# firechecking/CleanTransformer

Measured on AMD Instinct MI355X. Metric: SFT tokens/sec/step Bloom-560M bf16, higher is better.
Workload: dtype bf16

## Files before the change

cleantransformer_amd/_lib.py:

```python
from __future__ import annotations

import ctypes as C
import os

import torch

from ._build import LIB_PATH as _DEFAULT_LIB_PATH

LIB_PATH = os.environ.get("CTMI_LIB_PATH") or _DEFAULT_LIB_PATH

F32, BF16, F16 = 0, 1, 2
OPT_LEGACY_GRID = 4
OPT_SHADOW_F16 = 2
EPI_NONE, EPI_GELU, EPI_DGELU, EPI_RELU, EPI_DRELU, EPI_GELUG, EPI_MUL = 0, 1, 2, 3, 4, 5, 6
MT_MAX = 24
PROF_CLASSES = ("gemm_fwd", "gemm_dgrad", "gemm_wgrad", "lm_head", "attn_fwd", "attn_bwd", "layernorm", "loss", "optimizer", "reduce", "other")
ABI_VERSION = 16

vp, i64, i32, f32 = C.c_void_p, C.c_int64, C.c_int, C.c_float


class CtmiError(RuntimeError):
    pass


class AttnDesc(C.Structure):
    _fields_ = [(n, i64) for n in ("B", "nh", "Sq", "Sk", "hd",
                                   "q_bs", "q_hs", "q_rs", "k_bs", "k_hs", "k_rs",
                                   "v_bs", "v_hs", "v_rs", "o_bs", "o_hs", "o_rs",
                                   "am_b", "am_h", "am_q", "am_k")] + [("scale", f32), ("causal", i32), ("future_fill", f32), ("dropout_seed", C.c_uint32), ("dropout_p", f32), ("reserved_", i32)]


# ... 4 lines not shown
class WgradProblem(C.Structure):
    _fields_ = [("dy", vp), ("x", vp), ("dw", vp), ("db", vp), ("n_out", i64), ("n_in", i64), ("in_out", i32), ("pad_", i32)]


BLK_SLOTS = ("ln1", "mean1", "rstd1", "qkv", "att", "stat_m", "stat_l", "h1", "mean2", "rstd2", "ln2", "u", "g", "out")
BLK_QKV_BLOCKED, BLK_WGRAD_IN_OUT, BLK_W_IN_OUT = 1, 2, 4
BLK_PARAMS = ("ln1_w", "ln1_b", "wqkv", "bqkv", "wd", "bd", "ln2_w", "ln2_b", "w1", "b1", "w2", "b2")


class BloomBlock(C.Structure):
    _fields_ = [("B", i64), ("S", i64), ("H", i64), ("nh", i64), ("eps", f32), ("post_ln_res", i32), ("dtype", i32), ("flags", i32),
                ("attn_scale", f32), ("future_fill", f32)] + \
               [(n, vp) for n in BLK_PARAMS] + [(n, vp) for n in ("slopes", "kpos", "kvalid", "first_valid", "x", "slab")]


class BloomBlockGrads(C.Structure):
    _fields_ = [("dout", vp), ("dx", vp)] + [("d" + n, vp) for n in BLK_PARAMS] + \
               [("ws", vp), ("ws_bytes", i64), ("splitk_ws", vp), ("splitk_ws_bytes", i64), ("side_stream", vp),
                ("side_splitk_ws", vp), ("side_splitk_ws_bytes", i64), ("defer_join", i32)]


PROTOTYPES = {
    "ctmi_abi_version": (i32, []),
    "ctmi_last_error": (C.c_char_p, []),
    "ctmi_layernorm_fwd": (i32, [vp, vp, vp, vp, vp, vp, i64, i64, f32, i32, vp]),
    "ctmi_layernorm_bwd_ws": (i64, [i64, i64]),
    "ctmi_layernorm_bwd": (i32, [vp, vp, vp, vp, vp, vp, vp, vp, vp, i32, vp, i64, i64, i32, vp]),
    "ctmi_gemm": (i32, [vp, i64, i32, vp, i64, i32, vp, i64, i64, i64, i64, f32, i32, vp, vp, i32, vp, vp, i32, i32, vp, i64, vp]),
    "ctmi_set_launch_policy": (i32, [i32, i32]),
    "ctmi_get_launch_policy": (i32, [C.POINTER(i32), C.POINTER(i32)]),
    "ctmi_colsum": (i32, [vp, i64, vp, i32, vp, i64, i64, i32, vp]),
    "ctmi_colsum_ws": (i64, [i64, i64]),
    "ctmi_attn_fwd": (i32, [vp, vp, vp, vp, vp, vp, vp, vp, vp, vp, vp, C.POINTER(AttnDesc), i32, vp]),
    "ctmi_attn_bwd": (i32, [vp, vp, vp, vp, vp, vp, vp, vp, vp, vp, vp, vp, vp, vp, vp, vp, C.POINTER(AttnDesc), i32, vp]),
# ... 1 lines not shown
    "ctmi_mask_prep": (i32, [vp, vp, vp, vp, i64, i64, vp]),
    "ctmi_embed_fwd": (i32, [vp, vp, vp, i64, i64, i64, i32, vp, vp]),
    "ctmi_embed_bwd": (i32, [vp, vp, vp, i64, i64, i64, i32, f32, vp]),
    "ctmi_ce_fwd": (i32, [vp, i64, vp, vp, vp, vp, i64, i64, i64, i64, i64, i32, i64, i32, vp]),
    "ctmi_ce_bwd": (i32, [vp, i64, vp, vp, vp, vp, vp, i64, i64, i64, i64, i64, i64, i32, vp]),
    "ctmi_ce_fwd_bwd": (i32, [vp, i64, vp, vp, vp, vp, vp, i64, i64, i64, i64, i64, i64, i32, i64, f32, vp, i32, vp]),
    "ctmi_scale_if": (i32, [vp, i64, i64, i64, vp, f32, vp, i32, vp]),
    "ctmi_scale_if_passes": (i64, []),
    "ctmi_reduce_jobs": (i32, [C.POINTER(ReduceJob), i32, vp]),
    "ctmi_wgrad_grouped": (i32, [C.POINTER(WgradProblem), i32, i64, i32, vp, i64, vp]),
    "ctmi_bloom_block_layout": (i64, [i64, i64, i64, i64, i32, C.POINTER(i64)]),
    "ctmi_bloom_block_fwd": (i32, [C.POINTER(BloomBlock), vp]),
    "ctmi_bloom_block_bwd_ws": (i64, [i64, i64, i64, i64, i32]),
    "ctmi_bloom_block_wgrad_grouped": (i32, [i64, i64, i64, i32, i32]),
    "ctmi_bloom_block_bwd": (i32, [C.POINTER(BloomBlock), C.POINTER(BloomBlockGrads), vp]),
    "ctmi_ce_soft_fwd": (i32, [vp, i64, vp, i64, vp, vp, vp, vp, i64, i64, i32, i64, i32, vp]),
    "ctmi_ce_soft_bwd": (i32, [vp, i64, vp, i64, vp, vp, vp, vp, vp, i64, i64, i64, i32, vp]),
    "ctmi_ddp_unique_id": (C.c_int, [C.c_void_p]),
    "ctmi_ddp_create": (C.c_int, [C.c_void_p, C.c_int, C.c_int, C.c_int, C.POINTER(C.c_void_p)]),
    "ctmi_ddp_destroy": (C.c_int, [C.c_void_p]),
    "ctmi_ddp_all_reduce": (C.c_int, [C.c_void_p, C.c_void_p, C.c_int64, C.c_int, C.c_void_p]),
    "ctmi_ddp_all_gather": (C.c_int, [C.c_void_p, C.c_void_p, C.c_void_p, C.c_int64, C.c_void_p]),
    "ctmi_ddp_broadcast": (C.c_int, [C.c_void_p, C.c_void_p, C.c_int64, C.c_int, C.c_void_p]),
    "ctmi_ddp_wait": (C.c_int, [C.c_void_p, C.c_void_p]),
    "ctmi_dropout_hash": (C.c_uint32, [C.c_uint32]),
    "ctmi_dropout_keep_hash": (C.c_uint32, [C.c_uint32, C.c_uint32]),
    "ctmi_dropout_threshold": (C.c_uint32, [f32]),
    "ctmi_dropout": (i32, [vp, vp, vp, i64, f32, C.c_uint32, i32, vp]),
    "ctmi_adamw_step": (i32, [C.POINTER(vp), C.POINTER(vp), C.POINTER(vp), C.POINTER(vp), C.POINTER(vp), C.POINTER(i64),
                              i32, f32, f32, f32, f32, f32, i32, i32, i32, f32, vp]),
# ... 63 lines not shown
```

cleantransformer_amd/csrc/block.hip:

```cpp
#include "common.h"
#include <math.h>
#include <stdlib.h>
#include <mutex>

int ctmi_ln_bwd_parts_internal(const void* dy, const void* x, const float* w, const float* mean, const float* rstd,
                               const void* dres, void* dx, float* ws, int64_t rows, int64_t cols, int dtype, int want_sums,
                               int* nparts, int* ns, hipStream_t st);
int ctmi_colsum_parts_internal(const void* x, int64_t ld, float* ws, int64_t M, int64_t N, int dtype, int* parts_out, hipStream_t st);
bool ctmi_wgrad_grouped_ok(const ctmi_wgrad_problem* pr, int n, int64_t T, int dtype);
int ctmi_wgrad_grouped_ex(const ctmi_wgrad_problem* pr, int n, int64_t T, int dtype, void* workspace, int64_t workspace_bytes, void* stream, bool defer_reduce);
int ctmi_wgrad_tail(const ctmi_reduce_job* jobs, int count, hipStream_t st);
void ctmi_wgrad_pending_clear();
bool ctmi_wgrad_pending();

static inline int64_t al256(int64_t b) { return (b + 255) / 256 * 256; }

extern "C" int64_t ctmi_bloom_block_layout(int64_t B, int64_t S, int64_t H, int64_t nh, int dtype, int64_t* offs) {
    const int64_t T = B * S, e = dtype == CTMI_F32 ? 4 : 2;
    int64_t o = 0;
    auto put = [&](int slot, int64_t bytes) { if (offs) offs[slot] = o; o += al256(bytes); };
    put(CTMI_BLK_LN1, T * H * e);
    put(CTMI_BLK_MEAN1, T * 4);
    put(CTMI_BLK_RSTD1, T * 4);
    put(CTMI_BLK_QKV, T * 3 * H * e);
    put(CTMI_BLK_ATT, T * H * e);
// ... 135 lines not shown
}
}

extern "C" int ctmi_bloom_block_wgrad_grouped(int64_t B, int64_t S, int64_t H, int dtype, int flags) {
    if (B <= 0 || S <= 0 || H <= 0) return 0;
    const int io = (flags & CTMI_BLK_WGRAD_IN_OUT) ? 1 : 0;
    void* const al = reinterpret_cast<void*>(uintptr_t(256));
    float* const fa = reinterpret_cast<float*>(al);
    const ctmi_wgrad_problem wp[4] = {{al, al, fa, nullptr, H, 4 * H, io, 0}, {al, al, fa, io ? nullptr : fa, 4 * H, H, io, 0},
                                      {al, al, fa, nullptr, H, H, io, 0}, {al, al, fa, io ? nullptr : fa, 3 * H, H, io, 0}};
    return ctmi_wgrad_grouped_ok(wp, 4, B * S, dtype) ? 1 : 0;
}

extern "C" int64_t ctmi_bloom_block_bwd_ws(int64_t B, int64_t S, int64_t H, int64_t nh, int dtype) {
    return bwd_layout(B, S, H, nh, dtype, nullptr);
}

extern "C" int ctmi_bloom_block_bwd(const ctmi_bloom_block* b, const ctmi_bloom_block_grads* gr, void* stream) {
    RC(check_block(b, "bloom_block_bwd"));
    CTMI_REQUIRE(gr != nullptr && gr->dout && gr->dx && gr->ws, "bloom_block_bwd: null gradient pointer / workspace");
    CTMI_REQUIRE(gr->dln1_w && gr->dln1_b && gr->dwqkv && gr->dbqkv && gr->dwd && gr->dbd && gr->dln2_w && gr->dln2_b && gr->dw1 && gr->db1 &&
                 gr->dw2 && gr->db2, "bloom_block_bwd: null parameter-gradient pointer");
    const int64_t T = b->B * b->S, H = b->H, hd = H / b->nh;
    const int dt = b->dtype, e = dt == CTMI_F32 ? 4 : 2;
    int64_t woff[W_NSLOTS];
    const int64_t need = bwd_layout(b->B, b->S, H, b->nh, dt, woff);
    CTMI_REQUIRE(gr->ws_bytes >= need, "bloom_block_bwd: workspace too small (%lld < %lld bytes)", (long long)gr->ws_bytes, (long long)need);
    Slab s; s.base = reinterpret_cast<char*>(b->slab);
    ctmi_bloom_block_layout(b->B, b->S, H, b->nh, dt, s.off);
    char* wsb = reinterpret_cast<char*>(gr->ws);
// ... 6 lines not shown
    hipStream_t side = gr->side_stream ? as_stream(gr->side_stream) : nullptr;
    const bool two = side != nullptr && side != main_st;
    hipStream_t pst = two ? side : main_st;
    void* pws = two ? gr->side_splitk_ws : gr->splitk_ws;
    const int64_t pws_bytes = two ? gr->side_splitk_ws_bytes : gr->splitk_ws_bytes;
    auto fork = [&]() -> int {
        if (!two) return CTMI_OK;
        hipEvent_t ev = next_event();
        CTMI_HIP_OK(hipEventRecord(ev, main_st), "bloom_block_bwd: event record");
        CTMI_HIP_OK(hipStreamWaitEvent(side, ev, 0), "bloom_block_bwd: stream wait");
        return CTMI_OK;
    };

    ctmi_wgrad_pending_clear();
    ctmi_reduce_job jobs[CTMI_REDUCE_MAX_JOBS];
    int nj = 0;
    auto job = [&](const float* src, int64_t stride, int nparts, float* dst, int64_t n) {
        ctmi_reduce_job& J = jobs[nj++];
        J.src = src; J.dst = dst; J.n = n; J.part_stride = stride; J.nparts = nparts; J.accumulate = 0; J.alpha = 1.0f; J.pad_ = 0;
    };
    auto colsum_job = [&](const void* x, int64_t N, int slot, float* dst) -> int {
        int parts = 0;
        RC(ctmi_colsum_parts_internal(x, N, WF(slot), T, N, dt, &parts, pst));
        job(WF(slot), N, parts, dst, N);
        return CTMI_OK;
    };

    const void* dout = gr->dout;
    ctmi_wgrad_problem wp[4] = {
        {dout, s.at(CTMI_BLK_G), gr->dw2, nullptr, H, 4 * H, wio ? 1 : 0, 0},
        {W(W_DU), s.at(CTMI_BLK_LN2), gr->dw1, gr->db1, 4 * H, H, wio ? 1 : 0, 0},
        {W(W_DH1), s.at(CTMI_BLK_ATT), gr->dwd, nullptr, H, H, wio ? 1 : 0, 0},
        {W(W_DQKV), s.at(CTMI_BLK_LN1), gr->dwqkv, gr->dbqkv, 3 * H, H, wio ? 1 : 0, 0},
    };
    const int wp_cs[4] = {-1, W_CS_DU, -1, W_CS_DQKV};
    const bool grouped = ctmi_wgrad_grouped_ok(wp, 4, T, dt);
    int np2 = 0, ns2 = 2;
    auto out_bias_jobs = [&]() -> int {
        if (ns2 == 4 && !post) job(WF(W_LNP2) + 2 * H, ns2 * H, np2, gr->db2, H);
        else RC(colsum_job(dout, H, W_CS_DOUT, gr->db2));
        if (ns2 == 4) job(WF(W_LNP2) + 3 * H, ns2 * H, np2, gr->dbd, H);
        else RC(colsum_job(W(W_DH1), H, W_CS_DH1, gr->dbd));
        return CTMI_OK;
    };
    auto wgrad = [&](int i) -> int {
        if (grouped) return CTMI_OK;
        RC(fork());
        if (i == 2) RC(out_bias_jobs());
        const ctmi_wgrad_problem& p = wp[i];
        RC(linear_wgrad(p.dy, p.x, p.dw, T, p.n_out, p.n_in, dt, pws, pws_bytes, pst, wio));
        if (p.db) RC(colsum_job(p.dy, p.n_out, wp_cs[i], p.db));
// ... 7 lines not shown
        RC(ctmi_ln_bwd_parts_internal(W(W_DLN2), s.at(CTMI_BLK_H1), b->ln2_w, s.at<float>(CTMI_BLK_MEAN2), s.at<float>(CTMI_BLK_RSTD2),
                                      post ? nullptr : dout, W(W_DH1), WF(W_LNP2), T, H, dt, 1, &np2, &ns2, main_st));
        job(WF(W_LNP2), ns2 * H, np2, gr->dln2_w, H);
        job(WF(W_LNP2) + H, ns2 * H, np2, gr->dln2_b, H);
        RC(wgrad(2));
        RC(linear_dgrad(W(W_DH1), b->wd, W(W_DATT), T, H, H, CTMI_EPI_NONE, nullptr, nullptr, dt, gr->splitk_ws, gr->splitk_ws_bytes, main_st, w_io));
        const ctmi_attn_desc d = fused_qkv_desc(b);
        char* qkv = s.at<char>(CTMI_BLK_QKV);
        char* dqkv = reinterpret_cast<char*>(W(W_DQKV));
        RC(ctmi_attn_bwd(qkv, qkv + qkv_part(b, 1) * e, qkv + qkv_part(b, 2) * e, s.at(CTMI_BLK_ATT), W(W_DATT), s.at<float>(CTMI_BLK_STAT_M), s.at<float>(CTMI_BLK_STAT_L),
                         dqkv, dqkv + qkv_part(b, 1) * e, dqkv + qkv_part(b, 2) * e, WF(W_DELTA), b->slopes, b->kpos, b->kvalid, b->first_valid, nullptr, &d, dt, main_st));
        RC(wgrad(3));
        if (grouped) {
            RC(fork());
            RC(out_bias_jobs());
            RC(ctmi_wgrad_grouped_ex(wp, 4, T, dt, pws, pws_bytes, pst, !two));
        }
        const bool pend = ctmi_wgrad_pending();
        RC(linear_dgrad(dqkv, b->wqkv, W(W_DLN1), T, 3 * H, H, CTMI_EPI_NONE, nullptr, post ? W(W_DH1) : nullptr, dt, pend ? nullptr : gr->splitk_ws, pend ? 0 : gr->splitk_ws_bytes, main_st, w_io));
        int np1 = 0, ns1 = 2;
        RC(ctmi_ln_bwd_parts_internal(W(W_DLN1), b->x, b->ln1_w, s.at<float>(CTMI_BLK_MEAN1), s.at<float>(CTMI_BLK_RSTD1),
                                      post ? nullptr : W(W_DH1), gr->dx, WF(W_LNP1), T, H, dt, 0, &np1, &ns1, main_st));
        job(WF(W_LNP1), ns1 * H, np1, gr->dln1_w, H);
        job(WF(W_LNP1) + H, ns1 * H, np1, gr->dln1_b, H);
        return CTMI_OK;
    }();
    if (two && gr->defer_join && rc_launch == CTMI_OK) {
        RC(fork());
        RC(ctmi_reduce_jobs(jobs, nj, side));
        return CTMI_OK;
    }
    if (two) {
        hipEvent_t ev = next_event();
        const hipError_t e1 = hipEventRecord(ev, side);
        const hipError_t e2 = e1 == hipSuccess ? hipStreamWaitEvent(main_st, ev, 0) : e1;
        if (e2 != hipSuccess && rc_launch == CTMI_OK) { ctmi_set_error("bloom_block_bwd: joining the side stream: %s", hipGetErrorString(e2)); return CTMI_ERR_LAUNCH; }
    }
    if (rc_launch != CTMI_OK) { ctmi_wgrad_pending_clear(); return rc_launch; }
    RC(ctmi_wgrad_tail(jobs, nj, main_st));
    return CTMI_OK;
}
```

cleantransformer_amd/csrc/gemm.hip:

```cpp
#include "common.h"
#include "reduce_jobs.h"
#include <type_traits>
#include "mma.h"
#include "prof.h"
#include <atomic>
#ifndef CTMI_GEMM_PART
#define CTMI_GEMM_PART (-1)
#endif
#define CTMI_GEMM_HAS(p) (CTMI_GEMM_PART == -1 || CTMI_GEMM_PART == (p))

constexpr bool glds_k2(bool pp, int wm) { return pp && wm == 4; }
constexpr int glds_ring(bool pp, int wm, bool xlane = false) { return !pp ? 3 : (glds_k2(pp, wm) ? 6 : 4); }
constexpr int glds_patch_bytes(bool pp, int wm, bool xlane = false) { return (pp && !xlane && wm != 4) ? 4 * 8192 : 0; }


template <typename T> struct Tile;
template <> struct Tile<bf16_t> { static constexpr int BM = 128, BN = 128, BK = 64, PADK = 8, PADR = 8; };
template <> struct Tile<f16_t>  { static constexpr int BM = 128, BN = 128, BK = 64, PADK = 8, PADR = 8; };
template <> struct Tile<float>  { static constexpr int BM = 128, BN = 128, BK = 16, PADK = 4, PADR = 4; };

template <typename T, bool KMAJOR, int ROWS>
struct OpTile {
    static constexpr int BK = Tile<T>::BK;
    static constexpr int VEC = 16 / sizeof(T);
// ... 92 lines not shown
template <> __device__ __forceinline__ float OpTile<float, true, 128>::frag(const float* __restrict__ tile, int r16, int lane, int kofs) {
    return tile[kofs * PITCH + r16 + (lane & 15)];
}

struct GemmArgs {
    const void* A; const void* B; void* C;
    int64_t lda, ldb, ldc, M, N, K;
    float alpha; int beta;
    const float* bias; const void* residual; const void* aux_in; void* aux_out;
    int tiles_m, tiles_n, vec_c, vec8;
    int nt_c;
    int splits; int64_t k_per_split; float* slabs;
    int splitk_ok; float* ws; int64_t ws_bytes;
};

constexpr int WG_MAXP = 4;
struct GroupProb { const void* A; const void* B; float* C; float* cs; float* part; float* cspart; int64_t lda, ldb, ldc, M, N, csn; };
struct GroupedArgs : GemmArgs { GroupProb p[WG_MAXP]; const int4* items; int nitems; };
constexpr int WG_PART = 16, WG_COLSUM = 32, WG_HALF1 = 64, WG_COLSUMB = 128;
template <bool GRP, int WM, bool BSUM = false> struct GrpRegs { };
template <int WM> struct GrpRegs<true, WM, false> { f32x4 accs; bool cs_on; };
template <int WM> struct GrpRegs<true, WM, true> { f32x4 accs; bool cs_on; f32x4 accb[4]; bool csb_on; };
#define WG_ONES8 (std::is_same<T, f16_t>::value ? short8{0x3C00, 0x3C00, 0x3C00, 0x3C00, 0x3C00, 0x3C00, 0x3C00, 0x3C00} \
                                                : short8{0x3F80, 0x3F80, 0x3F80, 0x3F80, 0x3F80, 0x3F80, 0x3F80, 0x3F80})

template <typename TO> __device__ __forceinline__ void store4(TO* p, const float* v);
template <> __device__ __forceinline__ void store4<float>(float* p, const float* v) { *reinterpret_cast<float4*>(p) = make_float4(v[0], v[1], v[2], v[3]); }
template <> __device__ __forceinline__ void store4<bf16_t>(bf16_t* p, const float* v) { *reinterpret_cast<uint2*>(p) = make_uint2(pack_bf2(v[0], v[1]), pack_bf2(v[2], v[3])); }
template <> __device__ __forceinline__ void store4<f16_t>(f16_t* p, const float* v) { *reinterpret_cast<uint2*>(p) = make_uint2(pack_h2(v[0], v[1]), pack_h2(v[2], v[3])); }
template <typename TO> __device__ __forceinline__ void load4(const TO* p, float* v);
template <> __device__ __forceinline__ void load4<float>(const float* p, float* v) { float4 t = *reinterpret_cast<const float4*>(p); v[0] = t.x; v[1] = t.y; v[2] = t.z; v[3] = t.w; }
template <> __device__ __forceinline__ void load4<bf16_t>(const bf16_t* p, float* v) {
    uint2 t = *reinterpret_cast<const uint2*>(p);
    v[0] = __uint_as_float(t.x << 16); v[1] = __uint_as_float(t.x & 0xffff0000u); v[2] = __uint_as_float(t.y << 16); v[3] = __uint_as_float(t.y & 0xffff0000u);
// ... 1197 lines not shown
}

#if CTMI_GEMM_HAS(1)
int ctmi_gemm_bf16_nt(GemmArgs& g, int epi, bool fast, hipStream_t st) { return gemm_nt<bf16_t, bf16_t>(g, epi, fast, st); }
#endif
#if CTMI_GEMM_HAS(2)
int ctmi_gemm_bf16_nn(GemmArgs& g, int epi, bool fast, hipStream_t st) { return gemm_nn<bf16_t, bf16_t>(g, epi, fast, st); }
#endif
#if CTMI_GEMM_HAS(3)
int ctmi_gemm_bf16_tn(GemmArgs& g, int epi, bool fast, hipStream_t st) { return gemm_tn<bf16_t>(g, epi, fast, st); }

#include <map>
#include <mutex>
#include <vector>
namespace {
struct WgShape { int64_t M[WG_MAXP], N[WG_MAXP]; int cs[WG_MAXP]; int n; int64_t ksteps; int slots; int split;
    bool operator<(const WgShape& o) const {
        if (n != o.n) return n < o.n;
        if (ksteps != o.ksteps) return ksteps < o.ksteps;
        if (slots != o.slots) return slots < o.slots;
        if (split != o.split) return split < o.split;
        for (int i = 0; i < n; ++i) { if (M[i] != o.M[i]) return M[i] < o.M[i]; if (N[i] != o.N[i]) return N[i] < o.N[i]; if (cs[i] != o.cs[i]) return cs[i] < o.cs[i]; }
        return false;
    }
};
struct WgTable { int4* dev = nullptr; int nitems = 0, nsplit = 0; unsigned split_mask = 0; };
std::mutex g_wg_mu;
std::map<std::pair<int, WgShape>, WgTable> g_wg_tables;

inline int xcd_pos(int b, int L) {
    const int xcd = b & 7, q = L >> 3, r8 = L & 7;
    return (xcd < r8 ? xcd * (q + 1) : r8 * (q + 1) + (xcd - r8) * q) + (b >> 3);
}

void build_items(const WgShape& sh, std::vector<int4>& out, int& nitems, int& nsplit, unsigned& split_mask) {
    struct Tile { int p, m0, n0; };
    std::vector<Tile> tiles;
    for (int p = 0; p < sh.n; ++p) {
        const int tm = (int)(sh.M[p] / 128), tn = (int)(sh.N[p] / 256);
        for (int g0 = 0; g0 < tm; g0 += 8) {
            const int gm = std::min(8, tm - g0);
            for (int j = 0; j < tn; ++j)
                for (int i = 0; i < gm; ++i) tiles.push_back({p, (g0 + i) * 128, j * 256});
        }
    }
    const int nt = (int)tiles.size(), slots = sh.slots;
    const int ks = (int)sh.ksteps, h0 = ks / 2, h1 = ks - h0;
    int whole = nt;
    if (sh.split == 2 && ks >= 2) whole = 0;
    else if (sh.split == 1 && ks >= 2) { const int R = nt % slots; if (R > 0 && 2 * R <= slots) whole = nt - R; }
    split_mask = 0;
    auto csflag = [&](const Tile& t) { return sh.cs[t.p] == 1 ? (t.n0 == 0 ? WG_COLSUM : 0) : (sh.cs[t.p] == 2 ? (t.m0 == 0 ? WG_COLSUMB : 0) : 0); };
    auto item = [&](const Tile& t, int kb, int n, bool part) {
        const int cs = csflag(t);
        if (part) split_mask |= 1u << t.p;
        return make_int4(t.p | (part ? WG_PART : 0) | ((part && kb) ? WG_HALF1 : 0) | cs, t.m0, t.n0, kb | (n << 16));
    };
    std::vector<int4> lin;
    for (int t = 0; t < whole; ++t) lin.push_back(item(tiles[t], 0, ks, false));
    for (int t0 = whole; t0 < nt; t0 += 16) {
        const int t1 = std::min(nt, t0 + 16);
        for (int t = t0; t < t1; ++t) lin.push_back(item(tiles[t], 0, h0, true));
        for (int t = t0; t < t1; ++t) lin.push_back(item(tiles[t], h0, h1, true));
    }
    const int total = (int)lin.size();
    out.assign(total, make_int4(0, 0, 0, 0));
    for (int r0 = 0; r0 < total; r0 += slots) {
        const int L = std::min(slots, total - r0);
        for (int b = 0; b < L; ++b) out[r0 + b] = lin[r0 + xcd_pos(b, L)];
    }
    nitems = total; nsplit = nt - whole;
    for (int t = whole; t < nt; ++t) out.push_back(make_int4(tiles[t].p | csflag(tiles[t]), tiles[t].m0, tiles[t].n0, 0));
}
}

int ctmi_wgrad_group_mode() {
    static const int v = std::max(0, ctmi_env_int("CTMI_WGRAD_GROUP", 1));
    return v;
}

bool ctmi_wgrad_grouped_ok(const ctmi_wgrad_problem* pr, int n, int64_t T, int dtype) {
    if (ctmi_wgrad_group_mode() == 0 || !glds_enabled() || (dtype != CTMI_BF16 && dtype != CTMI_F16) || n < 1 || n > WG_MAXP || T < 64 || T % 32 != 0 || T / 32 > 0x7fff) return false;
    for (int i = 0; i < n; ++i) {
        const int64_t M = pr[i].in_out ? pr[i].n_in : pr[i].n_out, N = pr[i].in_out ? pr[i].n_out : pr[i].n_in;
        if (M <= 0 || N <= 0 || M % 128 != 0 || N % 256 != 0) return false;
        if (M * N >= (32LL << 20)) return false;
        if (!pr[i].dy || !pr[i].x || !pr[i].dw) return false;
        if ((((uintptr_t)pr[i].dy) | ((uintptr_t)pr[i].x) | ((uintptr_t)pr[i].dw)) & 15) return false;
// ... 9 lines not shown
    if (!g_wg_pending.valid) return ctmi_reduce_jobs(jobs, count, st);
    g_wg_pending.valid = false;
    if (st != g_wg_pending.st || count > CTMI_REDUCE_MAX_JOBS || count <= 0) {
        hipLaunchKernelGGL(wgrad_partials_reduce_k, dim3(4 * g_wg_pending.z.ntiles), dim3(256), 0, g_wg_pending.st, g_wg_pending.z);
        CTMI_CHECK_LAUNCH("wgrad_grouped_reduce");
        return ctmi_reduce_jobs(jobs, count, st);
    }
    ProfScope prof__(CTMI_PROF_REDUCE, st);
    ReduceJobs R;
    const int chunks = reduce_jobs_pack(jobs, count, R);
    if (chunks < 0) return CTMI_ERR_ARG;
    hipLaunchKernelGGL(wgrad_tail_k, dim3((unsigned)(4 * g_wg_pending.z.ntiles + chunks)), dim3(256), 0, st, g_wg_pending.z, R);
    CTMI_CHECK_LAUNCH("wgrad_tail");
    return CTMI_OK;
}
int ctmi_wgrad_grouped_ex(const ctmi_wgrad_problem* pr, int n, int64_t T, int dtype, void* workspace, int64_t workspace_bytes, void* stream, bool defer_reduce);
extern "C" int ctmi_wgrad_grouped(const ctmi_wgrad_problem* pr, int n, int64_t T, int dtype, void* workspace, int64_t workspace_bytes, void* stream) {
    return ctmi_wgrad_grouped_ex(pr, n, T, dtype, workspace, workspace_bytes, stream, false);
}
int ctmi_wgrad_grouped_ex(const ctmi_wgrad_problem* pr, int n, int64_t T, int dtype, void* workspace, int64_t workspace_bytes, void* stream, bool defer_reduce) {
    CTMI_REQUIRE(pr != nullptr, "wgrad_grouped: null problem list");
    if (!ctmi_wgrad_grouped_ok(pr, n, T, dtype)) {
        ctmi_set_error("wgrad_grouped: unsupported problem set (bf16 / fp16, <= %d problems, rows a multiple of 128 and columns of 256 of every gradient, T %% 32 == 0, "
                       "16-byte aligned operands and bias gradients; CTMI_WGRAD_GROUP != 0)", WG_MAXP);
        return CTMI_ERR_UNSUPPORTED;
    }
    hipStream_t st = as_stream(stream);
    ProfScope prof__(CTMI_PROF_GEMM_WGRAD, st);
    const int persist = shared_mode() ? 0 : 1;
    const int slots = (256 - reserved_cus()) / 8 * 8;
    WgShape sh = {};
    sh.n = n; sh.ksteps = T / 32; sh.slots = slots;
    const int mode = ctmi_wgrad_group_mode();
    sh.split = mode == 3 ? 0 : (mode == 2 ? 2 : 1);
    {
        int64_t need = 0;
        for (int i = 0; i < n; ++i) { const int64_t M = pr[i].in_out ? pr[i].n_in : pr[i].n_out, N = pr[i].in_out ? pr[i].n_out : pr[i].n_in; need += 2 * (M * N + std::max(M, N)) * 4 + 512; }
        if (sh.split != 0 && (workspace == nullptr || workspace_bytes < need || (((uintptr_t)workspace) & 15))) {
            static std::atomic<bool> said{false};
            if (!said.exchange(true))
                fprintf(stderr, "[ctmi355] wgrad_grouped: workspace of %lld bytes (need %lld, 16-byte aligned) — the tiles of the last partial round are NOT cut "
                                "in K-halves (same results, lower speed)\n", (long long)workspace_bytes, (long long)need);
            sh.split = 0;
        }
    }
    GroupedArgs g = {};
    bool bsum = false;
    g.M = 128; g.N = 256; g.K = T; g.k_per_split = T; g.splits = 1; g.alpha = 1.0f;
    for (int i = 0; i < n; ++i) {
// ... 138 lines not shown
```

cleantransformer_amd/models/modeling_bloom.py:

```python
from __future__ import annotations

import math
import os as _os
from typing import NamedTuple, Optional

import torch

from .. import _lib, ops, rng
from ..generation.generation_util import GenerationMixin
from ..transformer import LayerNorm

Tensor = torch.Tensor


class BloomConfig():

    def __init__(
            self,
            vocab_size=250880,
            hidden_size=64,
            n_layer=2,
            num_attention_heads=8,
            layer_norm_epsilon=1e-5,
            initializer_range=0.02,
# ... 84 lines not shown
                                   flags=spec.flags, attn_scale=spec.attn_scale, future_fill=spec.future_fill)
        ops.note_block_params(spec.mask, ps)
        grad = getattr(kv_out, "grad", True) and any(ctx.needs_input_grad)
        if grad:
            ctx.save_for_backward(x2, *ps, acts.slab)
            ctx.geo, ctx.spec, ctx.shape = acts.geometry(), spec, (B, S, H)
        kv = ops.LazyKV(acts, blocked=spec.kv_blocked, eager=not grad)
        if grad:
            ctx.kv = kv
        kv_out.append(kv)
        return acts.out.view(B, S, H)

    @staticmethod
    def backward(ctx, dout):
        if dout is None:
            return (None,) * (1 + _NP + 2)
        x2, *ps, slab = ctx.saved_tensors
        spec = ctx.spec
        B, S, H = ctx.shape
        dout2 = ops._c(dout.reshape(B * S, H))
        ctx.kv.release()
        side = _WGRAD_SIDE_STREAM if spec.side_stream_override else None
        defer = side is not False and x2.is_cuda and ops.params_allow_deferred_grads(ps, spec.mask)
        dx, g = ops.bloom_block_bwd(ops.BlockActs.rebuild(slab, ctx.geo), x2, ops.block_params(ps, x2.dtype), spec.mask, spec.slopes, spec.eps,
                                    spec.post_ln_res, dout2, use_side_stream=side, defer_join=defer)
        return (dx.view(B, S, H), *g, None, None)


def _lora_of(linear: torch.nn.Module):
    a = getattr(linear, "lora_A", None)
    return None if a is None else (a.weight, linear.lora_B.weight, float(linear.lora_scaling))


def _project(x2: Tensor, w_c: Tensor, bias: Tensor, res: Optional[Tensor], lora, p: float = 0.0, seed: int = 0):
    y = ops.linear_fwd(x2, w_c, bias, residual=None if p > 0.0 else res)
    xa = None
    if lora is not None:
        a, b, scaling = lora
        a_c, b_c = ops.compute_weight(a, x2.dtype), ops.compute_weight(b, x2.dtype)
        xa = ops.lora_project(x2, a_c, False, alpha=scaling)
# ... 444 lines not shown
```

cleantransformer_amd/ops.py:

```python
from __future__ import annotations

import contextlib
import os
import ctypes as C
import math
import threading
from typing import Optional, Tuple

import torch

from . import _lib
from ._lib import AttnDesc, BF16, F16, F32, check

Tensor = torch.Tensor


def _p(t: Optional[Tensor]):
    return None if t is None else C.c_void_p(t.data_ptr())


def _stream():
    return C.c_void_p(torch.cuda.current_stream().cuda_stream)


# ... 568 lines not shown


_GROUPED = {}
_WGRAD_STREAM_ENV = os.environ.get("CTMI_WGRAD_STREAM", "auto")


def block_wgrad_grouped(B: int, S: int, H: int, dtype: torch.dtype, flags: int = 0) -> bool:
    key = (B, S, H, dtype, flags)
    v = _GROUPED.get(key)
    if v is None:
        v = bool(_lib.load().ctmi_bloom_block_wgrad_grouped(B, S, H, dt_code(dtype), int(flags)))
        _GROUPED[key] = v
    return v


def bloom_block_bwd(acts: BlockActs, x2: Tensor, params, mask: Optional[MaskInfo], slopes: Optional[Tensor], eps: float,
                    post_ln_res: bool, dout2: Tensor, use_side_stream: Optional[bool] = None, defer_join: bool = False):
    _need_cuda(x2, dout2)
    B, S, H, nh = acts.B, acts.S, acts.H, acts.nh
    dev = x2.device
    if use_side_stream is None:
        use_side_stream = (_WGRAD_STREAM_ENV != "0") if _WGRAD_STREAM_ENV in ("0", "1") else not block_wgrad_grouped(B, S, H, x2.dtype, acts.flags)
    if torch.cuda.is_current_stream_capturing():
        use_side_stream = defer_join = False
    d = _lib.BloomBlock()
    _fill_block_desc(d, x2, params, mask, slopes, eps, post_ln_res, B, S, H, nh, acts.slab, acts.flags, acts.attn_scale, acts.future_fill)
    g = _lib.BloomBlockGrads()
    dx = torch.empty_like(x2)
    flip = bool(acts.flags & _lib.BLK_WGRAD_IN_OUT) != bool(acts.flags & _lib.BLK_W_IN_OUT)
    grads = [torch.empty(tuple(reversed(p.shape)) if (flip and p.dim() == 2) else p.shape, dtype=torch.float32, device=dev) for p in params]
    g.dout, g.dx = dout2.data_ptr(), dx.data_ptr()
    for name, t in zip(_lib.BLK_PARAMS, grads):
        setattr(g, "d" + name, t.data_ptr())
    defer_join = bool(defer_join and use_side_stream)
    main = torch.cuda.current_stream(dev)
    st = None
    slot = 0
    if defer_join:
        st = _DEFER.setdefault(dev, [0, {}])
        slot = st[0]
        st[0] ^= 1
        prev = st[1].get(slot)
        if prev is not None:
            main.wait_event(prev)
    elif dev in _DEFER and _DEFER[dev][1] and not torch.cuda.is_current_stream_capturing():
        for ev in _DEFER[dev][1].values():
            main.wait_event(ev)
        _DEFER[dev][1].clear()
    ws = _block_ws(dev, acts.lay.bwd_ws_bytes, slot)
    g.ws, g.ws_bytes = ws.data_ptr(), ws.numel()
    sk = _splitk_ws(dev)
    g.splitk_ws, g.splitk_ws_bytes = sk.data_ptr(), sk.numel() * 4
    if use_side_stream:
        side = side_stream(dev)
        with torch.cuda.stream(side):
            sk2 = _splitk_ws(dev)
        g.side_stream = side.cuda_stream
        g.side_splitk_ws, g.side_splitk_ws_bytes = sk2.data_ptr(), sk2.numel() * 4
    g.defer_join = int(defer_join)
    check(_lib.load().ctmi_bloom_block_bwd(C.byref(d), C.byref(g), _stream()), "bloom_block_bwd")
    if defer_join:
        ev = torch.cuda.Event()
        ev.record(side)
        st[1][slot] = ev
        acts.slab.record_stream(side)
        dout2.record_stream(side)
        for t in grads:
            t.record_stream(side)
        _LAST_DEFERRED_GRAD_PTRS[:] = [t.data_ptr() for t in grads]
        torch.autograd.Variable._execution_engine.queue_callback(lambda main=main, side=side: main.wait_stream(side))
    return dx, grads


def dropout(x: Tensor, p: float, seed: int, residual: Optional[Tensor] = None, out: Optional[Tensor] = None) -> Tensor:
    _need_cuda(x, residual)
# ... 385 lines not shown
```

include/ctmi355.h:

```cpp
#ifndef CTMI355_H
#define CTMI355_H

#include <stdint.h>

#ifdef __cplusplus
extern "C" {
#endif

#define CTMI_ABI_VERSION 16

enum ctmi_dtype { CTMI_F32 = 0, CTMI_BF16 = 1, CTMI_F16 = 2 };
enum ctmi_status { CTMI_OK = 0, CTMI_ERR_ARG = -1, CTMI_ERR_LAUNCH = -2, CTMI_ERR_UNSUPPORTED = -3 };

int ctmi_abi_version(void);
const char* ctmi_last_error(void);

int ctmi_layernorm_fwd(const void* x, const float* w, const float* b, void* y, float* mean, float* rstd,
                       int64_t rows, int64_t cols, float eps, int dtype, void* stream);
int64_t ctmi_layernorm_bwd_ws(int64_t rows, int64_t cols);
int ctmi_layernorm_bwd(const void* dy, const void* x, const float* w, const float* mean, const float* rstd,
                       const void* dres, void* dx, float* dw, float* db, int accumulate, float* ws,
                       int64_t rows, int64_t cols, int dtype, void* stream);

enum ctmi_epilogue { CTMI_EPI_NONE = 0, CTMI_EPI_GELU = 1, CTMI_EPI_DGELU = 2, CTMI_EPI_RELU = 3, CTMI_EPI_DRELU = 4,
// ... 144 lines not shown
    float eps; int32_t post_ln_res;
    int32_t dtype;
    int32_t flags;
    float attn_scale;
    float future_fill;
    const float *ln1_w, *ln1_b; const void* wqkv; const float* bqkv; const void* wd; const float* bd;
    const float *ln2_w, *ln2_b; const void* w1; const float* b1; const void* w2; const float* b2;
    const float* slopes;
    const float* kpos; const int32_t* kvalid; const int32_t* first_valid;
    const void* x;
    void* slab;
} ctmi_bloom_block;
int64_t ctmi_bloom_block_layout(int64_t B, int64_t S, int64_t H, int64_t nh, int dtype, int64_t* offsets );
int ctmi_bloom_block_fwd(const ctmi_bloom_block* blk , void* stream);

typedef struct ctmi_bloom_block_grads {
    const void* dout;
    void* dx;
    float *dln1_w, *dln1_b, *dwqkv, *dbqkv, *dwd, *dbd, *dln2_w, *dln2_b, *dw1, *db1, *dw2, *db2;
    void* ws; int64_t ws_bytes;
    void* splitk_ws; int64_t splitk_ws_bytes;
    void* side_stream;
    void* side_splitk_ws; int64_t side_splitk_ws_bytes;
    int defer_join;
} ctmi_bloom_block_grads;
int64_t ctmi_bloom_block_bwd_ws(int64_t B, int64_t S, int64_t H, int64_t nh, int dtype);
int ctmi_bloom_block_wgrad_grouped(int64_t B, int64_t S, int64_t H, int dtype, int flags);
int ctmi_bloom_block_bwd(const ctmi_bloom_block* blk , const ctmi_bloom_block_grads* gr , void* stream);

int ctmi_lora_project(const void* x, int64_t ldx, const void* w, int64_t ldw, int w_kmajor, void* out, int64_t ldo,
                      int64_t T, int64_t K, int64_t r, float alpha, int dtype, void* stream);
int ctmi_lora_expand_add(const void* xa, int64_t ldxa, const void* w, int64_t ldw, int w_kmajor, void* y, int64_t ldy,
                         int64_t T, int64_t N, int64_t r, int dtype, void* stream);
int64_t ctmi_lora_wgrad_ws(int64_t T, int64_t P, int64_t Q);
int ctmi_lora_wgrad(const void* l, int64_t ldl, const void* r, int64_t ldr, float* out, int64_t ldo, int64_t T, int64_t P, int64_t Q,
                    float alpha, float* ws, int64_t ws_bytes, int dtype, void* stream);

int ctmi_probe(int which, const float* in , float* out , void* stream);
int ctmi_clock_probe(int mfma_iters, unsigned long long* out , void* stream);
int ctmi_probe_dyn_lds(int64_t bytes, unsigned* out , void* stream);

#ifdef __cplusplus
}
// ... 3 lines not shown
```

Before: 230,400.

## Pair weight-gradient grouped GEMMs of two consecutive Bloom blocks into one launch

During backward, a block's four weight-gradient problems can be parked instead of launched. The next block's backward then runs them together with its own as one eight-problem grouped GEMM, with no K split, and merges both blocks' partial-row reduce jobs into one tail launch. The aim is fuller use of the GPU's compute units by the wgrad kernel and fewer launches and split-K reductions. The cost is extra bookkeeping: an autograd callback that flushes any leftover parked record, held references to keep buffers alive, and a dedicated workspace slot.

```diff
diff --git a/cleantransformer_amd/_lib.py b/cleantransformer_amd/_lib.py
--- a/cleantransformer_amd/_lib.py
+++ b/cleantransformer_amd/_lib.py
@@ -15,7 +15,7 @@
 EPI_NONE, EPI_GELU, EPI_DGELU, EPI_RELU, EPI_DRELU, EPI_GELUG, EPI_MUL = 0, 1, 2, 3, 4, 5, 6
 MT_MAX = 24
 PROF_CLASSES = ("gemm_fwd", "gemm_dgrad", "gemm_wgrad", "lm_head", "attn_fwd", "attn_bwd", "layernorm", "loss", "optimizer", "reduce", "other")
-ABI_VERSION = 16
+ABI_VERSION = 17
 
 vp, i64, i32, f32 = C.c_void_p, C.c_int64, C.c_int, C.c_float
 
@@ -50,10 +50,15 @@
                [(n, vp) for n in BLK_PARAMS] + [(n, vp) for n in ("slopes", "kpos", "kvalid", "first_valid", "x", "slab")]
 
 
+class BloomBlockPending(C.Structure):
+    _fields_ = [("wp", WgradProblem * 4), ("jobs", ReduceJob * 8), ("njobs", i32), ("dtype", i32), ("T", i64)]
+
+
 class BloomBlockGrads(C.Structure):
     _fields_ = [("dout", vp), ("dx", vp)] + [("d" + n, vp) for n in BLK_PARAMS] + \
                [("ws", vp), ("ws_bytes", i64), ("splitk_ws", vp), ("splitk_ws_bytes", i64), ("side_stream", vp),
-                ("side_splitk_ws", vp), ("side_splitk_ws_bytes", i64), ("defer_join", i32)]
+                ("side_splitk_ws", vp), ("side_splitk_ws_bytes", i64), ("defer_join", i32),
+                ("park", C.POINTER(BloomBlockPending)), ("paired", C.POINTER(BloomBlockPending))]
 
 
 PROTOTYPES = {
@@ -85,6 +90,7 @@
     "ctmi_bloom_block_bwd_ws": (i64, [i64, i64, i64, i64, i32]),
     "ctmi_bloom_block_wgrad_grouped": (i32, [i64, i64, i64, i32, i32]),
     "ctmi_bloom_block_bwd": (i32, [C.POINTER(BloomBlock), C.POINTER(BloomBlockGrads), vp]),
+    "ctmi_bloom_block_wgrad_flush": (i32, [C.POINTER(BloomBlockPending), vp, i64, vp]),
     "ctmi_ce_soft_fwd": (i32, [vp, i64, vp, i64, vp, vp, vp, vp, i64, i64, i32, i64, i32, vp]),
     "ctmi_ce_soft_bwd": (i32, [vp, i64, vp, i64, vp, vp, vp, vp, vp, i64, i64, i64, i32, vp]),
     "ctmi_ddp_unique_id": (C.c_int, [C.c_void_p]),
diff --git a/cleantransformer_amd/csrc/block.hip b/cleantransformer_amd/csrc/block.hip
--- a/cleantransformer_amd/csrc/block.hip
+++ b/cleantransformer_amd/csrc/block.hip
@@ -8,7 +8,7 @@
                                int* nparts, int* ns, hipStream_t st);
 int ctmi_colsum_parts_internal(const void* x, int64_t ld, float* ws, int64_t M, int64_t N, int dtype, int* parts_out, hipStream_t st);
 bool ctmi_wgrad_grouped_ok(const ctmi_wgrad_problem* pr, int n, int64_t T, int dtype);
-int ctmi_wgrad_grouped_ex(const ctmi_wgrad_problem* pr, int n, int64_t T, int dtype, void* workspace, int64_t workspace_bytes, void* stream, bool defer_reduce);
+int ctmi_wgrad_grouped_ex(const ctmi_wgrad_problem* pr, int n, int64_t T, int dtype, void* workspace, int64_t workspace_bytes, void* stream, bool defer_reduce, bool no_cut);
 int ctmi_wgrad_tail(const ctmi_reduce_job* jobs, int count, hipStream_t st);
 void ctmi_wgrad_pending_clear();
 bool ctmi_wgrad_pending();
@@ -174,6 +174,14 @@
 
 extern "C" int64_t ctmi_bloom_block_bwd_ws(int64_t B, int64_t S, int64_t H, int64_t nh, int dtype) {
     return bwd_layout(B, S, H, nh, dtype, nullptr);
+}
+
+extern "C" int ctmi_bloom_block_wgrad_flush(const ctmi_bloom_block_pending* rec, void* workspace, int64_t workspace_bytes, void* stream) {
+    CTMI_REQUIRE(rec != nullptr && rec->njobs >= 0 && rec->njobs <= CTMI_BLK_PENDING_MAX_JOBS, "bloom_block_wgrad_flush: bad record");
+    ctmi_wgrad_pending_clear();
+    const int rc = ctmi_wgrad_grouped_ex(rec->wp, 4, rec->T, rec->dtype, workspace, workspace_bytes, stream, true, false);
+    if (rc != CTMI_OK) { ctmi_wgrad_pending_clear(); return rc; }
+    return ctmi_wgrad_tail(rec->jobs, rec->njobs, as_stream(stream));
 }
 
 extern "C" int ctmi_bloom_block_bwd(const ctmi_bloom_block* b, const ctmi_bloom_block_grads* gr, void* stream) {
@@ -210,6 +218,7 @@
 
     ctmi_wgrad_pending_clear();
     ctmi_reduce_job jobs[CTMI_REDUCE_MAX_JOBS];
+    static_assert(2 * CTMI_BLK_PENDING_MAX_JOBS <= CTMI_REDUCE_MAX_JOBS, "two blocks' partial-row jobs are one reduce launch");
     int nj = 0;
     auto job = [&](const float* src, int64_t stride, int nparts, float* dst, int64_t n) {
         ctmi_reduce_job& J = jobs[nj++];
@@ -231,6 +240,20 @@
     };
     const int wp_cs[4] = {-1, W_CS_DU, -1, W_CS_DQKV};
     const bool grouped = ctmi_wgrad_grouped_ok(wp, 4, T, dt);
+    CTMI_REQUIRE(!(gr->park && gr->paired), "bloom_block_bwd: park and paired exclude each other");
+    CTMI_REQUIRE(!gr->park || (grouped && !two), "bloom_block_bwd: park needs the grouped weight-gradient path and no side stream");
+    ctmi_wgrad_problem wp8[8];
+    const ctmi_bloom_block_pending* pair = gr->paired;
+    if (pair) {
+        CTMI_REQUIRE(pair->njobs >= 0 && pair->njobs <= CTMI_BLK_PENDING_MAX_JOBS, "bloom_block_bwd: bad paired record");
+        for (int i = 0; i < 4; ++i) { wp8[i] = pair->wp[i]; wp8[4 + i] = wp[i]; }
+        if (!grouped || two || pair->T != T || pair->dtype != dt || !ctmi_wgrad_grouped_ok(wp8, 8, T, dt)) {
+            RC(ctmi_bloom_block_wgrad_flush(pair, gr->splitk_ws, gr->splitk_ws_bytes, main_st));
+            pair = nullptr;
+        } else {
+            for (int i = 0; i < pair->njobs; ++i) jobs[nj++] = pair->jobs[i];
+        }
+    }
     int np2 = 0, ns2 = 2;
     auto out_bias_jobs = [&]() -> int {
         if (ns2 == 4 && !post) job(WF(W_LNP2) + 2 * H, ns2 * H, np2, gr->db2, H);
@@ -268,7 +291,8 @@
         if (grouped) {
             RC(fork());
             RC(out_bias_jobs());
-            RC(ctmi_wgrad_grouped_ex(wp, 4, T, dt, pws, pws_bytes, pst, !two));
+            if (pair) RC(ctmi_wgrad_grouped_ex(wp8, 8, T, dt, nullptr, 0, pst, false, true));
+            else if (!gr->park) RC(ctmi_wgrad_grouped_ex(wp, 4, T, dt, pws, pws_bytes, pst, !two, false));
         }
         const bool pend = ctmi_wgrad_pending();
         RC(linear_dgrad(dqkv, b->wqkv, W(W_DLN1), T, 3 * H, H, CTMI_EPI_NONE, nullptr, post ? W(W_DH1) : nullptr, dt, pend ? nullptr : gr->splitk_ws, pend ? 0 : gr->splitk_ws_bytes, main_st, w_io));
@@ -291,6 +315,14 @@
         if (e2 != hipSuccess && rc_launch == CTMI_OK) { ctmi_set_error("bloom_block_bwd: joining the side stream: %s", hipGetErrorString(e2)); return CTMI_ERR_LAUNCH; }
     }
     if (rc_launch != CTMI_OK) { ctmi_wgrad_pending_clear(); return rc_launch; }
+    if (gr->park) {
+        ctmi_bloom_block_pending* pk = gr->park;
+        CTMI_REQUIRE(nj <= CTMI_BLK_PENDING_MAX_JOBS, "bloom_block_bwd: %d partial-row jobs do not fit a parked record", nj);
+        for (int i = 0; i < 4; ++i) pk->wp[i] = wp[i];
+        for (int i = 0; i < nj; ++i) pk->jobs[i] = jobs[i];
+        pk->njobs = nj; pk->dtype = dt; pk->T = T;
+        return CTMI_OK;
+    }
     RC(ctmi_wgrad_tail(jobs, nj, main_st));
     return CTMI_OK;
 }
diff --git a/cleantransformer_amd/csrc/gemm.hip b/cleantransformer_amd/csrc/gemm.hip
--- a/cleantransformer_amd/csrc/gemm.hip
+++ b/cleantransformer_amd/csrc/gemm.hip
@@ -130,10 +130,9 @@
     int splitk_ok; float* ws; int64_t ws_bytes;
 };
 
-constexpr int WG_MAXP = 4;
+#include "wgrad_items.h"
 struct GroupProb { const void* A; const void* B; float* C; float* cs; float* part; float* cspart; int64_t lda, ldb, ldc, M, N, csn; };
 struct GroupedArgs : GemmArgs { GroupProb p[WG_MAXP]; const int4* items; int nitems; };
-constexpr int WG_PART = 16, WG_COLSUM = 32, WG_HALF1 = 64, WG_COLSUMB = 128;
 template <bool GRP, int WM, bool BSUM = false> struct GrpRegs { };
 template <int WM> struct GrpRegs<true, WM, false> { f32x4 accs; bool cs_on; };
 template <int WM> struct GrpRegs<true, WM, true> { f32x4 accs; bool cs_on; f32x4 accb[4]; bool csb_on; };
@@ -1361,64 +1360,9 @@
 #include <mutex>
 #include <vector>
 namespace {
-struct WgShape { int64_t M[WG_MAXP], N[WG_MAXP]; int cs[WG_MAXP]; int n; int64_t ksteps; int slots; int split;
-    bool operator<(const WgShape& o) const {
-        if (n != o.n) return n < o.n;
-        if (ksteps != o.ksteps) return ksteps < o.ksteps;
-        if (slots != o.slots) return slots < o.slots;
-        if (split != o.split) return split < o.split;
-        for (int i = 0; i < n; ++i) { if (M[i] != o.M[i]) return M[i] < o.M[i]; if (N[i] != o.N[i]) return N[i] < o.N[i]; if (cs[i] != o.cs[i]) return cs[i] < o.cs[i]; }
-        return false;
-    }
-};
 struct WgTable { int4* dev = nullptr; int nitems = 0, nsplit = 0; unsigned split_mask = 0; };
 std::mutex g_wg_mu;
 std::map<std::pair<int, WgShape>, WgTable> g_wg_tables;
-
-inline int xcd_pos(int b, int L) {
-    const int xcd = b & 7, q = L >> 3, r8 = L & 7;
-    return (xcd < r8 ? xcd * (q + 1) : r8 * (q + 1) + (xcd - r8) * q) + (b >> 3);
-}
-
-void build_items(const WgShape& sh, std::vector<int4>& out, int& nitems, int& nsplit, unsigned& split_mask) {
-    struct Tile { int p, m0, n0; };
-    std::vector<Tile> tiles;
-    for (int p = 0; p < sh.n; ++p) {
-        const int tm = (int)(sh.M[p] / 128), tn = (int)(sh.N[p] / 256);
-        for (int g0 = 0; g0 < tm; g0 += 8) {
-            const int gm = std::min(8, tm - g0);
-            for (int j = 0; j < tn; ++j)
-                for (int i = 0; i < gm; ++i) tiles.push_back({p, (g0 + i) * 128, j * 256});
-        }
-    }
-    const int nt = (int)tiles.size(), slots = sh.slots;
-    const int ks = (int)sh.ksteps, h0 = ks / 2, h1 = ks - h0;
-    int whole = nt;
-    if (sh.split == 2 && ks >= 2) whole = 0;
-    else if (sh.split == 1 && ks >= 2) { const int R = nt % slots; if (R > 0 && 2 * R <= slots) whole = nt - R; }
-    split_mask = 0;
-    auto csflag = [&](const Tile& t) { return sh.cs[t.p] == 1 ? (t.n0 == 0 ? WG_COLSUM : 0) : (sh.cs[t.p] == 2 ? (t.m0 == 0 ? WG_COLSUMB : 0) : 0); };
-    auto item = [&](const Tile& t, int kb, int n, bool part) {
-        const int cs = csflag(t);
-        if (part) split_mask |= 1u << t.p;
-        return make_int4(t.p | (part ? WG_PART : 0) | ((part && kb) ? WG_HALF1 : 0) | cs, t.m0, t.n0, kb | (n << 16));
-    };
-    std::vector<int4> lin;
-    for (int t = 0; t < whole; ++t) lin.push_back(item(tiles[t], 0, ks, false));
-    for (int t0 = whole; t0 < nt; t0 += 16) {
-        const int t1 = std::min(nt, t0 + 16);
-        for (int t = t0; t < t1; ++t) lin.push_back(item(tiles[t], 0, h0, true));
-        for (int t = t0; t < t1; ++t) lin.push_back(item(tiles[t], h0, h1, true));
-    }
-    const int total = (int)lin.size();
-    out.assign(total, make_int4(0, 0, 0, 0));
-    for (int r0 = 0; r0 < total; r0 += slots) {
-        const int L = std::min(slots, total - r0);
-        for (int b = 0; b < L; ++b) out[r0 + b] = lin[r0 + xcd_pos(b, L)];
-    }
-    nitems = total; nsplit = nt - whole;
-    for (int t = whole; t < nt; ++t) out.push_back(make_int4(tiles[t].p | csflag(tiles[t]), tiles[t].m0, tiles[t].n0, 0));
-}
 }
 
 int ctmi_wgrad_group_mode() {
@@ -1458,11 +1402,12 @@
     CTMI_CHECK_LAUNCH("wgrad_tail");
     return CTMI_OK;
 }
-int ctmi_wgrad_grouped_ex(const ctmi_wgrad_problem* pr, int n, int64_t T, int dtype, void* workspace, int64_t workspace_bytes, void* stream, bool defer_reduce);
+int ctmi_wgrad_grouped_ex(const ctmi_wgrad_problem* pr, int n, int64_t T, int dtype, void* workspace, int64_t workspace_bytes, void* stream, bool defer_reduce, bool no_cut);
 extern "C" int ctmi_wgrad_grouped(const ctmi_wgrad_problem* pr, int n, int64_t T, int dtype, void* workspace, int64_t workspace_bytes, void* stream) {
-    return ctmi_wgrad_grouped_ex(pr, n, T, dtype, workspace, workspace_bytes, stream, false);
-}
-int ctmi_wgrad_grouped_ex(const ctmi_wgrad_problem* pr, int n, int64_t T, int dtype, void* workspace, int64_t workspace_bytes, void* stream, bool defer_reduce) {
+    if (n > 4) { ctmi_set_error("wgrad_grouped: %d problems (at most 4 per call)", n); return CTMI_ERR_UNSUPPORTED; }
+    return ctmi_wgrad_grouped_ex(pr, n, T, dtype, workspace, workspace_bytes, stream, false, false);
+}
+int ctmi_wgrad_grouped_ex(const ctmi_wgrad_problem* pr, int n, int64_t T, int dtype, void* workspace, int64_t workspace_bytes, void* stream, bool defer_reduce, bool no_cut) {
     CTMI_REQUIRE(pr != nullptr, "wgrad_grouped: null problem list");
     if (!ctmi_wgrad_grouped_ok(pr, n, T, dtype)) {
         ctmi_set_error("wgrad_grouped: unsupported problem set (bf16 / fp16, <= %d problems, rows a multiple of 128 and columns of 256 of every gradient, T %% 32 == 0, "
@@ -1476,7 +1421,7 @@
     WgShape sh = {};
     sh.n = n; sh.ksteps = T / 32; sh.slots = slots;
     const int mode = ctmi_wgrad_group_mode();
-    sh.split = mode == 3 ? 0 : (mode == 2 ? 2 : 1);
+    sh.split = (mode == 3 || no_cut) ? 0 : (mode == 2 ? 2 : 1);
     {
         int64_t need = 0;
         for (int i = 0; i < n; ++i) { const int64_t M = pr[i].in_out ? pr[i].n_in : pr[i].n_out, N = pr[i].in_out ? pr[i].n_out : pr[i].n_in; need += 2 * (M * N + std::max(M, N)) * 4 + 512; }
diff --git a/cleantransformer_amd/csrc/wgrad_items.h b/cleantransformer_amd/csrc/wgrad_items.h
--- /dev/null
+++ b/cleantransformer_amd/csrc/wgrad_items.h
@@ -0,0 +1,68 @@
+#pragma once
+#include <stdint.h>
+#include <algorithm>
+#include <vector>
+#if !defined(__HIPCC__) && !defined(__HIP__)
+struct int4 { int x, y, z, w; };
+static inline int4 make_int4(int x, int y, int z, int w) { return int4{x, y, z, w}; }
+#endif
+
+constexpr int WG_MAXP = 8;
+constexpr int WG_PART = 16, WG_COLSUM = 32, WG_HALF1 = 64, WG_COLSUMB = 128;
+static_assert(WG_MAXP <= WG_PART && (WG_MAXP & (WG_MAXP - 1)) == 0, "the problem index is masked out of a work item's x word");
+
+struct WgShape { int64_t M[WG_MAXP], N[WG_MAXP]; int cs[WG_MAXP]; int n; int64_t ksteps; int slots; int split;
+    bool operator<(const WgShape& o) const {
+        if (n != o.n) return n < o.n;
+        if (ksteps != o.ksteps) return ksteps < o.ksteps;
+        if (slots != o.slots) return slots < o.slots;
+        if (split != o.split) return split < o.split;
+        for (int i = 0; i < n; ++i) { if (M[i] != o.M[i]) return M[i] < o.M[i]; if (N[i] != o.N[i]) return N[i] < o.N[i]; if (cs[i] != o.cs[i]) return cs[i] < o.cs[i]; }
+        return false;
+    }
+};
+
+inline int xcd_pos(int b, int L) {
+    const int xcd = b & 7, q = L >> 3, r8 = L & 7;
+    return (xcd < r8 ? xcd * (q + 1) : r8 * (q + 1) + (xcd - r8) * q) + (b >> 3);
+}
+
+inline void build_items(const WgShape& sh, std::vector<int4>& out, int& nitems, int& nsplit, unsigned& split_mask) {
+    struct Tile { int p, m0, n0; };
+    std::vector<Tile> tiles;
+    for (int p = 0; p < sh.n; ++p) {
+        const int tm = (int)(sh.M[p] / 128), tn = (int)(sh.N[p] / 256);
+        for (int g0 = 0; g0 < tm; g0 += 8) {
+            const int gm = std::min(8, tm - g0);
+            for (int j = 0; j < tn; ++j)
+                for (int i = 0; i < gm; ++i) tiles.push_back({p, (g0 + i) * 128, j * 256});
+        }
+    }
+    const int nt = (int)tiles.size(), slots = sh.slots;
+    const int ks = (int)sh.ksteps, h0 = ks / 2, h1 = ks - h0;
+    int whole = nt;
+    if (sh.split == 2 && ks >= 2) whole = 0;
+    else if (sh.split == 1 && ks >= 2) { const int R = nt % slots; if (R > 0 && 2 * R <= slots) whole = nt - R; }
+    split_mask = 0;
+    auto csflag = [&](const Tile& t) { return sh.cs[t.p] == 1 ? (t.n0 == 0 ? WG_COLSUM : 0) : (sh.cs[t.p] == 2 ? (t.m0 == 0 ? WG_COLSUMB : 0) : 0); };
+    auto item = [&](const Tile& t, int kb, int n, bool part) {
+        const int cs = csflag(t);
+        if (part) split_mask |= 1u << t.p;
+        return make_int4(t.p | (part ? WG_PART : 0) | ((part && kb) ? WG_HALF1 : 0) | cs, t.m0, t.n0, kb | (n << 16));
+    };
+    std::vector<int4> lin;
+    for (int t = 0; t < whole; ++t) lin.push_back(item(tiles[t], 0, ks, false));
+    for (int t0 = whole; t0 < nt; t0 += 16) {
+        const int t1 = std::min(nt, t0 + 16);
+        for (int t = t0; t < t1; ++t) lin.push_back(item(tiles[t], 0, h0, true));
+        for (int t = t0; t < t1; ++t) lin.push_back(item(tiles[t], h0, h1, true));
+    }
+    const int total = (int)lin.size();
+    out.assign(total, make_int4(0, 0, 0, 0));
+    for (int r0 = 0; r0 < total; r0 += slots) {
+        const int L = std::min(slots, total - r0);
+        for (int b = 0; b < L; ++b) out[r0 + b] = lin[r0 + xcd_pos(b, L)];
+    }
+    nitems = total; nsplit = nt - whole;
+    for (int t = whole; t < nt; ++t) out.push_back(make_int4(tiles[t].p | csflag(tiles[t]), tiles[t].m0, tiles[t].n0, 0));
+}
diff --git a/cleantransformer_amd/models/modeling_bloom.py b/cleantransformer_amd/models/modeling_bloom.py
--- a/cleantransformer_amd/models/modeling_bloom.py
+++ b/cleantransformer_amd/models/modeling_bloom.py
@@ -122,6 +122,7 @@
     @staticmethod
     def backward(ctx, dout):
         if dout is None:
+            ops.flush_parked_wgrad()
             return (None,) * (1 + _NP + 2)
         x2, *ps, slab = ctx.saved_tensors
         spec = ctx.spec
@@ -129,9 +130,15 @@
         dout2 = ops._c(dout.reshape(B * S, H))
         ctx.kv.release()
         side = _WGRAD_SIDE_STREAM if spec.side_stream_override else None
-        defer = side is not False and x2.is_cuda and ops.params_allow_deferred_grads(ps, spec.mask)
-        dx, g = ops.bloom_block_bwd(ops.BlockActs.rebuild(slab, ctx.geo), x2, ops.block_params(ps, x2.dtype), spec.mask, spec.slopes, spec.eps,
-                                    spec.post_ln_res, dout2, use_side_stream=side, defer_join=defer)
+        late = x2.is_cuda and ops.params_allow_deferred_grads(ps, spec.mask)
+        defer = side is not False and late
+        pair_ok = side is not True and late and all(ctx.needs_input_grad[1:1 + _NP])
+        try:
+            dx, g = ops.bloom_block_bwd(ops.BlockActs.rebuild(slab, ctx.geo), x2, ops.block_params(ps, x2.dtype), spec.mask, spec.slopes, spec.eps,
+                                        spec.post_ln_res, dout2, use_side_stream=side, defer_join=defer, **({"pair_ok": True} if pair_ok else {}))
+        except BaseException:
+            ops.drop_parked_wgrad()
+            raise
         return (dx.view(B, S, H), *g, None, None)
 
 
diff --git a/cleantransformer_amd/ops.py b/cleantransformer_amd/ops.py
--- a/cleantransformer_amd/ops.py
+++ b/cleantransformer_amd/ops.py
@@ -606,8 +606,43 @@
     return v
 
 
+_WGRAD_PAIR = os.environ.get("CTMI_WGRAD_PAIR", "1") != "0"
+_PARKED = None
+PAIR_COUNTS = {"pairs": 0, "alone": 0}
+
+
+class _Parked:
+    __slots__ = ("rec", "key", "task", "dev", "main", "keep")
+
+
+def _graph_task() -> int:
+    return torch._C._current_graph_task_id()
+
+
+def drop_parked_wgrad() -> None:
+    global _PARKED
+    _PARKED = None
+
+
+def flush_parked_wgrad(only_task: Optional[int] = None) -> None:
+    global _PARKED
+    pk = _PARKED
+    if pk is None or (only_task is not None and pk.task != only_task):
+        return
+    _PARKED = None
+    with torch.cuda.device(pk.dev):
+        with torch.cuda.stream(pk.main):
+            sk = _splitk_ws(pk.dev)
+            check(_lib.load().ctmi_bloom_block_wgrad_flush(C.byref(pk.rec), sk.data_ptr(), sk.numel() * 4, pk.main.cuda_stream), "bloom_block_wgrad_flush")
+        cur = torch.cuda.current_stream(pk.dev)
+        if cur != pk.main:
+            cur.wait_stream(pk.main)
+    PAIR_COUNTS["alone"] += 1
+
+
 def bloom_block_bwd(acts: BlockActs, x2: Tensor, params, mask: Optional[MaskInfo], slopes: Optional[Tensor], eps: float,
-                    post_ln_res: bool, dout2: Tensor, use_side_stream: Optional[bool] = None, defer_join: bool = False):
+                    post_ln_res: bool, dout2: Tensor, use_side_stream: Optional[bool] = None, defer_join: bool = False, pair_ok: bool = False):
+    global _PARKED
     _need_cuda(x2, dout2)
     B, S, H, nh = acts.B, acts.S, acts.H, acts.nh
     dev = x2.device
@@ -626,6 +661,20 @@
         setattr(g, "d" + name, t.data_ptr())
     defer_join = bool(defer_join and use_side_stream)
     main = torch.cuda.current_stream(dev)
+    pair_key = None
+    if pair_ok and _WGRAD_PAIR and not use_side_stream and acts.flags == 0 and block_wgrad_grouped(B, S, H, x2.dtype, acts.flags):
+        pair_key = (dev, main.cuda_stream, B, S, H, nh, x2.dtype, bool(post_ln_res), _graph_task())
+    partner = _PARKED
+    if partner is not None and partner.key != pair_key:
+        flush_parked_wgrad()
+        partner = None
+    park = None
+    if partner is not None:
+        _PARKED = None
+        g.paired = C.pointer(partner.rec)
+    elif pair_key is not None:
+        park = _lib.BloomBlockPending()
+        g.park = C.pointer(park)
     st = None
     slot = 0
     if defer_join:
@@ -639,7 +688,7 @@
         for ev in _DEFER[dev][1].values():
             main.wait_event(ev)
         _DEFER[dev][1].clear()
-    ws = _block_ws(dev, acts.lay.bwd_ws_bytes, slot)
+    ws = _block_ws(dev, acts.lay.bwd_ws_bytes, 2 if park is not None else slot)
     g.ws, g.ws_bytes = ws.data_ptr(), ws.numel()
     sk = _splitk_ws(dev)
     g.splitk_ws, g.splitk_ws_bytes = sk.data_ptr(), sk.numel() * 4
@@ -651,6 +700,14 @@
         g.side_splitk_ws, g.side_splitk_ws_bytes = sk2.data_ptr(), sk2.numel() * 4
     g.defer_join = int(defer_join)
     check(_lib.load().ctmi_bloom_block_bwd(C.byref(d), C.byref(g), _stream()), "bloom_block_bwd")
+    if partner is not None:
+        PAIR_COUNTS["pairs"] += 1
+    elif park is not None:
+        pk = _Parked()
+        pk.rec, pk.key, pk.task, pk.dev, pk.main = park, pair_key, pair_key[-1], dev, main
+        pk.keep = (dout2, acts.slab, ws, [t.untyped_storage() for t in grads])
+        _PARKED = pk
+        torch.autograd.Variable._execution_engine.queue_callback(lambda task=pk.task: flush_parked_wgrad(task))
     if defer_join:
         ev = torch.cuda.Event()
         ev.record(side)
diff --git a/include/ctmi355.h b/include/ctmi355.h
--- a/include/ctmi355.h
+++ b/include/ctmi355.h
@@ -7,7 +7,7 @@
 extern "C" {
 #endif
 
-#define CTMI_ABI_VERSION 16
+#define CTMI_ABI_VERSION 17
 
 enum ctmi_dtype { CTMI_F32 = 0, CTMI_BF16 = 1, CTMI_F16 = 2 };
 enum ctmi_status { CTMI_OK = 0, CTMI_ERR_ARG = -1, CTMI_ERR_LAUNCH = -2, CTMI_ERR_UNSUPPORTED = -3 };
@@ -182,6 +182,13 @@
 int64_t ctmi_bloom_block_layout(int64_t B, int64_t S, int64_t H, int64_t nh, int dtype, int64_t* offsets );
 int ctmi_bloom_block_fwd(const ctmi_bloom_block* blk , void* stream);
 
+#define CTMI_BLK_PENDING_MAX_JOBS 8
+typedef struct ctmi_bloom_block_pending {
+    ctmi_wgrad_problem wp[4];
+    ctmi_reduce_job jobs[CTMI_BLK_PENDING_MAX_JOBS];
+    int32_t njobs; int32_t dtype; int64_t T;
+} ctmi_bloom_block_pending;
+
 typedef struct ctmi_bloom_block_grads {
     const void* dout;
     void* dx;
@@ -191,10 +198,13 @@
     void* side_stream;
     void* side_splitk_ws; int64_t side_splitk_ws_bytes;
     int defer_join;
+    ctmi_bloom_block_pending* park;
+    const ctmi_bloom_block_pending* paired;
 } ctmi_bloom_block_grads;
 int64_t ctmi_bloom_block_bwd_ws(int64_t B, int64_t S, int64_t H, int64_t nh, int dtype);
 int ctmi_bloom_block_wgrad_grouped(int64_t B, int64_t S, int64_t H, int dtype, int flags);
 int ctmi_bloom_block_bwd(const ctmi_bloom_block* blk , const ctmi_bloom_block_grads* gr , void* stream);
+int ctmi_bloom_block_wgrad_flush(const ctmi_bloom_block_pending* rec , void* workspace, int64_t workspace_bytes, void* stream);
 
 int ctmi_lora_project(const void* x, int64_t ldx, const void* w, int64_t ldw, int w_kmajor, void* out, int64_t ldo,
                       int64_t T, int64_t K, int64_t r, float alpha, int dtype, void* stream);
```

Result: no change. 232,700, median of 6 (+1.0%).
